# potsawee/tokenize-audio

Hardware: AMD Instinct MI355X
Metric: audio-sec encoded/sec (Mimi 8-codebook, 24 kHz) (higher is better)
Workload: dtype f16x3 (fp32-emulating: 2 fp16 planes per operand, 3 products, fp32 accumulate; RVQ distances fp32); 1 GPU; LibriTTS-R-style batch encode (configs[1]): batch=32 x 10 s @ 24 kHz resident in HBM, K=8 codebooks, 1 encode per step per GPU; global_batch=32, num_quantizers=8, parallelism=utterance round-robin x1 (no collective), gemm_precision=f16x3

## Files before the change

tokenize-audio_amd/csrc/engine.cpp:

```cpp
#include <hip/hip_runtime.h>

#include <algorithm>
#include <cmath>
#include <cstdarg>
#include <cstdio>
#include <cstdlib>
#include <cstring>
#include <fstream>
#include <map>
#include <memory>
#include <mutex>
#include <string>
#include <tuple>
#include <unordered_map>
#include <vector>

#include "../../include/mimi_hip.h"
#include "host_io.h"
#include "kernels.h"

using namespace mimi;

static thread_local std::string g_last_error;

// ... 242 lines not shown
        int ws_gen = 0, rope_gen = 0;
        hipGraph_t g = nullptr;
        hipGraphExec_t x = nullptr;
        uint64_t used = 0;
        unsigned* chain_flag = nullptr;
        size_t chain_clear = 0;
    };
    static constexpr int kMaxGraphs = 8;
    struct Lane {
        void* ws = nullptr;
        size_t ws_bytes = 0;
        int ws_gen = 0;
        hipEvent_t ws_free = nullptr;
        unsigned* amax_dev = nullptr;
        unsigned* amax_red = nullptr;
        void** io_dev = nullptr;
        std::vector<Graph> graphs;
        std::map<std::tuple<int, int64_t, int>, int> graph_seen;
        hipStream_t stream = nullptr;
        hipEvent_t in_ready = nullptr;
        int tickets = 0;
        int64_t encodes = 0;
        bool excl = false;
    };
    static constexpr int kLanes = 2;
    Lane lanes[kLanes];
    Lane* ln = &lanes[0];
    int lanes_opt = 1;
    bool graphs_enabled = true;
    bool capturing = false;
    size_t cap_chain_clear = 0;
    hipStream_t cap_stream = nullptr;
    int rope_gen = 0;
    uint64_t graph_clock = 0;
    int64_t graph_replays = 0, graph_captures = 0;

    bool taps = false;
    int stage0_fused = 1;
    int ln_fused = 1;
    int rvq_form = 0;
    int ln_rpw = 1;
    int rvq_xcd = 1;
    int rvq_chain = 1;
    bool chain_ok = false;
    unsigned* chain_flag = nullptr;
    int rvq_chain_fault = 0;
    int64_t chain_reruns = 0;
    int qkv_attn = 1;
    int qkv_attn_xcd = 1;
    int attn_band_split = 1;
    int sc1_out = 2;
    int fc1_cg = 1;
    int gemm256 = 3;
    int res1_form = 1;
    int res1_stream = 1;
    struct Tap {
        float* d = nullptr;
        size_t cap = 0;
        int64_t dims[3] = {0, 0, 0};
    };
    std::map<std::string, Tap> tapmap;

    bool decode_enabled = false;
    DevConv dec_first, dec_last;
    std::vector<DevConv> dec_up;
    std::vector<DevConv> dec_res3, dec_res1;
    std::vector<DevXfmr> dxf;
    float* outproj = nullptr;
    float* upsample_w = nullptr;
    void* dws = nullptr;
    size_t dws_bytes = 0;
    unsigned* dec_flag = nullptr;
    unsigned* dec_flag_host = nullptr;
};

static int dev_alloc(mimi_engine* e, void** p, size_t bytes) {
    hipError_t err = hipMalloc(p, bytes);
    if (err != hipSuccess) {
        (void)hipGetLastError();
        return set_err(err == hipErrorOutOfMemory ? MIMI_ERR_OUT_OF_MEMORY : MIMI_ERR_HIP, "hipMalloc(%zu): %s",
                       bytes, hipGetErrorString(err));
    }
    e->allocations.push_back(*p);
    return MIMI_OK;
}

static int upload(mimi_engine* e, float** dst, const std::vector<float>& host) {
    int rc = dev_alloc(e, reinterpret_cast<void**>(dst), host.size() * sizeof(float));
    if (rc) return rc;
    HIP_TRY(hipMemcpy(*dst, host.data(), host.size() * sizeof(float), hipMemcpyHostToDevice));
    return MIMI_OK;
}

static uint16_t f2bf_rne(float f) {
    uint32_t u;
    std::memcpy(&u, &f, 4);
    u += 0x7FFF + ((u >> 16) & 1);
    return (uint16_t)(u >> 16);
}
static float bf2f(uint16_t h) {
    const uint32_t u = (uint32_t)h << 16;
    float f;
    std::memcpy(&f, &u, 4);
    return f;
}

// ... 1002 lines not shown
                ra.hamax = ha.amax;
            }
            if (si == 1 && h16) {
                const Act xa = new_act("s1.x"), ha = new_act("s1.h");
                ra.wh16 = e->res1_h16;
                ra.xscale = xa.scale;
                ra.hscale = ha.scale;
                ra.unscale1 = 1.0f / (xa.scale * e->res1_wsc[0]);
                ra.unscale2 = 1.0f / (ha.scale * e->res1_wsc[1]);
                ra.xamax = xa.amax;
                ra.hamax = ha.amax;
                ra.form = e->res1_form;
            }
            if (rg && !(h16 && (si == 0 || si == 1))) return set_err(MIMI_ERR_UNSUPPORTED, "ragged: fp16 blocks only");
            const double H = C / c.compress;
            const double BT = rows_of(si, (double)B * T);
            const double fl = 2.0 * BT * (3.0 * C * H + H * C) + (si == 0 ? 2.0 * BT * C * c.kernel_size : 0.0);
            const DevConv& dc0 = e->down[0];
            bool t1_ceil = p.T[1] == (T + 3) / 4;
            if (rg)
                for (int b = 0; b < B; ++b) t1_ceil = t1_ceil && rg->plan[b].T[1] == (rg->plan[b].T[0] + 3) / 4;
            if (si == 0 && h16 && e->stage0_fused && C == 64 && dc0.cin == 64 && dc0.cout == 128 &&
                dc0.k == 8 && dc0.stride == 4 && dc0.wh && dc0.b && t1_ceil) {
                ra.wdown = dc0.wh;
                ra.bdown = dc0.b;
                ra.unscale_d = 1.0f / (yact.scale * dc0.wscale);
                ra.xout = w.x;
                ra.T1 = p.T[1];
                ra.yp = e->taps ? w.y : nullptr;
                LAUNCH_TRY(launch_stage0_fused(ra, s, &kname), "stage 0 + down conv 0");
                const double BT1 = rows_of(1, (double)B * p.T[1]);
                const double fld = 2.0 * BT1 * 128.0 * 512.0;
                const double by = BT * 4 + BT1 * 128 * 4 + (3.0 * C * H + H * C) * 4 + 128.0 * 512 * 4;
                rec.mark("res_down_s0", fl + fld, by, kname);
                if ((rc = save_tap_planes(e, "res0_elu", w.y, ns, B, T, C, s, yact.scale))) return rc;
                if ((rc = save_tap_planes(e, "down0", w.x, 0, B, p.T[1], 2 * C, s, 0.0f))) return rc;
                C *= 2;
                continue;
            }
            LAUNCH_TRY(launch_resblock(C, ra, s, &kname), "resblock");
            snprintf(nm, sizeof nm, "res_s%d", si);
            const double by = BT * 4 * (si == 0 ? 1 + C : 2 * C) + (3.0 * C * H + H * C) * 4;
            rec.mark(nm, fl, by, kname);
        } else {
            const int Hh = C / c.compress;
            GemmArgs a3 = conv_args(e->res3[si], nullptr, T, nullptr, T, B);
            planes_in(a3, w.xe, (long long)B * T * C);
            use_h(a3, e->res3[si].wh, e->res3[si].wscale, xeact);
            a3.Cp = w.h;
            a3.c_pstride = (long long)B * T * Hh;
            if (rg) a3.a_rows = a3.m_rows = dT[si];
            hact = new_act(nmf("h%d", si));
            out_act(a3, hact);
            LAUNCH_TRY(launch_gemm(ROLE_RES3P, a3, s, &kname, prec), "res3");
            snprintf(nm, sizeof nm, "res3_s%d", si);
            rec.mark(nm, gemm_flops(a3) * rows_of(si, (double)B * T) / ((double)B * T), gemm_bytes(a3, false), kname);
            GemmArgs a1 = conv_args(e->res1[si], nullptr, T, nullptr, T, B);
            planes_in(a1, w.h, (long long)B * T * Hh);
            use_h(a1, e->res1[si].wh, e->res1[si].wscale, hact);
            a1.R = w.x;
            a1.Cp = w.y;
            a1.c_pstride = (long long)B * T * C;
            if (rg) a1.a_rows = a1.m_rows = dT[si];
            yact = new_act(nmf("y%d", si));
            out_act(a1, yact);
            if (h16 && e->res1_stream && res1_stream_ok(a1) && (e->res1_stream == 2 || a1.K == 128))
                LAUNCH_TRY(launch_res1_stream(a1, s, &kname), "res1 stream");
            else
                LAUNCH_TRY(launch_gemm(ROLE_RES1P, a1, s, &kname, prec), "res1");
            snprintf(nm, sizeof nm, "res1_s%d", si);
            rec.mark(nm, gemm_flops(a1) * rows_of(si, (double)B * T) / ((double)B * T), gemm_bytes(a1, true), kname);
        }
        snprintf(nm, sizeof nm, "res%d_elu", si);
        if ((rc = save_tap_planes(e, nm, w.y, ns, B, T, C, s, yact.scale))) return rc;
        const bool last = si == c.num_ratios - 1;
        const bool next_unf = ns && !last && si + 1 >= mimi_engine::kUnfuseFrom;
        GemmArgs ad = conv_args(e->down[si], w.y, T, w.x, p.T[si + 1], B);
        int role = last ? ROLE_DOWN_ELU : ROLE_DOWN;
        if (ns) {
            planes_in(ad, w.y, (long long)B * T * C);
            use_h(ad, e->down[si].wh, e->down[si].wscale, yact);
            if (last) {
                ad.Cp = w.x;
                ad.c_pstride = (long long)B * p.T[si + 1] * 2 * C;
                ad.C = nullptr;
                xact = new_act("x_last");
                out_act(ad, xact);
            } else if (next_unf) {
                ad.Cp = w.xe;
                ad.c_pstride = (long long)B * p.T[si + 1] * 2 * C;
                role = ROLE_DOWN_XE;
                xeact = new_act(nmf("xe%d", si + 1));
                out_act(ad, xeact);
            }
        }
        if (rg) {
            ad.a_rows = dT[si];
            ad.m_rows = dT[si + 1];
        }
        LAUNCH_TRY(launch_gemm(role, ad, s, &kname, prec, rg ? 0 : e->gemm256), "down");
        snprintf(nm, sizeof nm, "down_s%d", si);
        rec.mark(nm, gemm_flops(ad) * rows_of(si + 1, (double)B * p.T[si + 1]) / ((double)B * p.T[si + 1]),
                 gemm_bytes(ad, false), kname);
        snprintf(nm, sizeof nm, last ? "down%d_elu" : "down%d", si);
        if ((rc = save_tap_planes(e, nm, w.x, last ? ns : 0, B, p.T[si + 1], 2 * C, s, last ? xact.scale : 0.0f)))
            return rc;
        C *= 2;
    }
    const int64_t T = p.frames25;
    const int Hd = c.hidden_size;
    GemmArgs af = conv_args(e->final_conv, w.x, p.T[c.num_ratios], w.t0, T, B);
    if (ns) planes_in(af, w.x, (long long)B * p.T[c.num_ratios] * C);
    use_h(af, e->final_conv.wh, e->final_conv.wscale, xact);
    if (rg) {
        af.a_rows = dT[c.num_ratios];
        af.m_rows = dT25;
        af.c_boff = dToff;
    }
    LAUNCH_TRY(launch_gemm(ROLE_FINAL, af, s, &kname, prec), "final");
    const double rT25 = rows_of(5, (double)B * p.frames25) / ((double)B * p.frames25);
    rec.mark("final", gemm_flops(af) * rT25, gemm_bytes(af, false), kname);
    const int64_t rows = rg ? rg->R : (int64_t)B * T;
    const int64_t tapB = rg ? 1 : B, tapT = rg ? rg->R : T;
    if ((rc = save_tap(e, "encoder", w.t0, tapB, tapT, Hd, s))) return rc;
    const int H = c.num_attention_heads, Dh = c.head_dim;
    const bool ds_planes = h16 && e->ds_fix && e->inproj_h && c.downsample_kernel == 4 && c.downsample_stride == 2;
    Act dsin, dsouta;
    double att_flops = 0;
    auto att_fl = [&](int64_t Tn) {
        double f = 0;
        for (int64_t i = 0; i < Tn; ++i) f += 4.0 * Dh * std::min<int64_t>(i + 1, c.sliding_window);
        return f * H;
    };
    if (rg) {
        for (const auto& pb : rg->plan) att_flops += att_fl(pb.frames25);
    } else {
        att_flops = att_fl(T) * B;
    }
    for (int l = 0; l < c.num_hidden_layers; ++l) {
        const DevXfmr& x = e->xf[l];
        const long long nact = rows * Hd;
        Act t1a = new_act(nmf("xf%d.ln1", l));
        if (ln_check_free(t1a, x.ln1_bound)) t1a.amax = nullptr;
        auto ln_into = [&](GemmArgs& g, int role, const float* lw, const float* lb, const Act& act) {
            if (!h16 || e->ln_fused < (role == ROLE_QKV ? 2 : 1) || !gemm_ln_prologue_ok(role, g, prec, rg ? 0 : e->gemm256)) return false;
            if (role == ROLE_QKV) g.ln_tile = e->ln_fused - 2;
            g.ln_x = w.t0;
            g.ln_g = lw;
            g.ln_b = lb;
            g.ln_eps = c.norm_eps;
            g.ln_scale = act.scale;
            g.ln_amax = act.amax;
            return true;
// ... 1394 lines not shown
    delete e;
}

extern "C" int mimi_set_precision(mimi_engine* e, int32_t mode) {
    if (!e) return set_err(MIMI_ERR_INVALID_ARGUMENT, "null engine");
    if (mode < MIMI_PRECISION_F32 || mode > MIMI_PRECISION_F16X3)
        return set_err(MIMI_ERR_INVALID_ARGUMENT, "precision mode %d", mode);
    std::lock_guard<std::mutex> lk(e->mu);
    if (e->precision != mode) {
        HIP_TRY(hipSetDevice(e->device));
        drain_lanes(e);
    }
    e->precision = mode;
    return MIMI_OK;
}

extern "C" int mimi_set_graphs(mimi_engine* e, int32_t enable) {
    if (!e) return set_err(MIMI_ERR_INVALID_ARGUMENT, "null engine");
    std::lock_guard<std::mutex> lk(e->mu);
    HIP_TRY(hipSetDevice(e->device));
    e->graphs_enabled = enable != 0;
    if (!enable) drop_graphs(e, true);
    return MIMI_OK;
}

extern "C" int64_t mimi_graph_replays(const mimi_engine* e) { return e ? e->graph_replays : -1; }

extern "C" int64_t mimi_graph_captures(const mimi_engine* e) { return e ? e->graph_captures : -1; }

extern "C" int64_t mimi_lane_encodes(const mimi_engine* e, int32_t lane) {
    return e && lane >= 0 && lane < mimi_engine::kLanes ? e->lanes[lane].encodes : -1;
}

struct EngineOption {
    const char* key;
    int mimi_engine::*field;
    unsigned allowed;
    const char* values;
};
static const EngineOption kEngineOptions[] = {
    {"stage0_fused", &mimi_engine::stage0_fused, 0x3u, "0 or 1"},
    {"rvq_form", &mimi_engine::rvq_form, 0x7fu, "0..6"},
    {"ln_rpw", &mimi_engine::ln_rpw, 0x117u, "0, 1, 2, 4 or 8"},
    {"rvq_xcd", &mimi_engine::rvq_xcd, 0x3u, "0 or 1"},
    {"rvq_chain", &mimi_engine::rvq_chain, 0x3u, "0 or 1"},
    {"rvq_chain_fault", &mimi_engine::rvq_chain_fault, 0x7u, "0, 1 or 2"},
    {"sc1_out", &mimi_engine::sc1_out, 0xffu, "0..7"},
    {"ln_fused", &mimi_engine::ln_fused, 0x1fu, "0 .. 4"},
    {"qkv_attn", &mimi_engine::qkv_attn, 0x7u, "0, 1 or 2"},
    {"qkv_attn_xcd", &mimi_engine::qkv_attn_xcd, 0x3u, "0 or 1"},
    {"attn_band_split", &mimi_engine::attn_band_split, 0x7u, "0, 1 or 2"},
    {"fc1_cg", &mimi_engine::fc1_cg, 0x17u, "0, 1, 2 or 4"},
    {"gemm256", &mimi_engine::gemm256, 0xffu, "0..7"},
    {"res1_form", &mimi_engine::res1_form, 0x3u, "0 or 1"},
    {"res1_stream", &mimi_engine::res1_stream, 0x7u, "0, 1 or 2"},
    {"lanes", &mimi_engine::lanes_opt, 0x7u, "0, 1 or 2"},
};

extern "C" int mimi_set_option(mimi_engine* e, const char* key, int64_t value) {
    if (!e || !key) return set_err(MIMI_ERR_INVALID_ARGUMENT, "null engine or key");
    std::lock_guard<std::mutex> lk(e->mu);
    for (const EngineOption& o : kEngineOptions) {
        if (strcmp(key, o.key)) continue;
        if (value < 0 || value > 31 || !((o.allowed >> value) & 1u))
            return set_err(MIMI_ERR_INVALID_ARGUMENT, "%s %lld (%s)", key, (long long)value, o.values);
        HIP_TRY(hipSetDevice(e->device));
        drain_lanes(e);
        if (e->*o.field != (int)value) drop_graphs(e, true);
        e->*o.field = (int)value;
        return MIMI_OK;
    }
    return set_err(MIMI_ERR_INVALID_ARGUMENT, "unknown option '%s'", key);
}

extern "C" int mimi_act_scales(mimi_engine* e, int32_t max_n, char* names, float* scales, float* last_max,
                               int32_t* n) {
    if (!e) return set_err(MIMI_ERR_INVALID_ARGUMENT, "null engine");
    std::lock_guard<std::mutex> lk(e->mu);
    int i = 0;
    for (const auto& kv : e->slot_of) {
        const int slot = kv.second;
        if (i >= max_n) break;
        if (names) {
            std::strncpy(names + 64 * i, kv.first.c_str(), 63);
            names[64 * i + 63] = 0;
        }
        if (scales) scales[i] = slot < (int)e->act_scale.size() ? e->act_scale[slot] : 0.0f;
        if (last_max) last_max[i] = slot < (int)e->last_amax.size() ? e->last_amax[slot] : -1.0f;
        ++i;
    }
    if (n) *n = i;
    return MIMI_OK;
}

extern "C" int mimi_get_precision(const mimi_engine* e) { return e ? e->precision : -1; }

extern "C" int mimi_calibrate(mimi_engine* e) {
    if (!e) return set_err(MIMI_ERR_INVALID_ARGUMENT, "null engine");
    if (!e->finalized) return set_err(MIMI_ERR_STATE, "mimi_finalize has not been called");
    std::lock_guard<std::mutex> lk(e->mu);
    if (e->calibrated) return MIMI_OK;
    HIP_TRY(hipSetDevice(e->device));
    (void)hipGetLastError();
    return calibrate_scales(e);
}

// ... 117 lines not shown
```

tokenize-audio_amd/csrc/gemm.hip:

```cpp
#include <algorithm>
#include <cstdio>
#include <cstdlib>


#include "gemm_planes.h"
#include "gemm_planes256.h"

#ifndef MIMI_QKV_V
#define MIMI_QKV_V 1
#endif
#ifndef MIMI_FC1_V
#define MIMI_FC1_V 0
#endif
#ifndef MIMI_SMALL16_32W
#define MIMI_SMALL16_32W 1
#endif
#ifndef MIMI_SMALL16_32
#define MIMI_SMALL16_32 15
#endif


namespace mimi {

template <int BM, int BN, int WM, int WN, int BK, int NBUF, bool NFAST, bool ELU_IN, int PAD, int EPI, int TAG>
// ... 210 lines not shown
            return run_planes<32, 32, 1, 2, 2, MIMI_DOWN_SMALL_ST, EPI, OUTP, TAG, 4, 32, 16, FL_PAIR | FL_KG2, true>(a, s);
        return run_planes<64, 64, 2, 2, 2, 4, EPI, OUTP, TAG, 4, 32, 16, FL_PAIR | FL_KG2, true>(a, s);
    }
    if (pair_ok(a) && tiles(a, 256, 128) < kSmallGrid)
        return run_planes<64, 64, 2, 2, 2, MIMI_DOWN_SMALL2_ST, EPI, OUTP, TAG, 4, 32, 16, FL_PAIR, true>(a, s);
    constexpr int PF = OUTP == 0 ? FL_PF : 0;
    if (pair_ok(a)) return run_planes<256, 128, 4, 2, 2, 2, EPI, OUTP, TAG, 4, 32, 16, FL_PAIR | FL_PERSIST | PF, true>(a, s);
    return run_planes<256, 128, 4, 2, 2, 3, EPI, OUTP, TAG, 0, 32, 16, 0, true>(a, s);
}

#ifndef MIMI_SMALL_ST
#define MIMI_SMALL_ST 4
#endif
#ifndef MIMI_LNA_ST
#define MIMI_LNA_ST 4
#endif
template <int EPI, int OUTP, int TAG, int BN0, int BM1, int BN1, int WM1, int WN1, int BN2, int WN2, int ST = MIMI_SMALL_ST,
          int FL = 0, int BM0 = 64, int WN0 = 2>
static hipError_t run_small_h16(const GemmArgs& a, hipStream_t s) {
    if (tiles(a, BM0, BN0) >= 256) return run_planes<BM0, BN0, 2, WN0, 2, ST, EPI, OUTP, TAG, 4, 32, 16, FL, true>(a, s);
    if (tiles(a, BM1, BN1) >= 256) return run_planes<BM1, BN1, WM1, WN1, 2, ST, EPI, OUTP, TAG, 4, 32, 16, FL, true>(a, s);
    return run_planes<16, BN2, 1, WN2, 2, ST, EPI, OUTP, TAG, 4, 32, 16, FL, true>(a, s);
}

bool gemm_ln_prologue_ok(int role, const GemmArgs& a, int precision, int g256) {
    if (role == ROLE_FC1 && (g256 & 4)) return false;
    return precision == PREC_F16X3 && (role == ROLE_QKV || role == ROLE_FC1) && a.K == 512 && a.a_rs == 512 &&
           a.a_off == 0 && !a.a_rows && !a.m_rows && !a.a_boff && tiles(a, 128, 128) < kSmallGrid;
}

static hipError_t dispatch_planes(int role, const GemmArgs& a, hipStream_t s) {
    const int prec = g_prec;
    if (prec != PREC_BF16X6 && prec != PREC_BF16X3 && prec != PREC_F16X3) return hipErrorInvalidValue;
    if (a.ln_x) {
        if (!gemm_ln_prologue_ok(role, a, prec) || !a.ln_g || !a.ln_b || !(a.ln_scale > 0.0f)) return hipErrorInvalidValue;
        if (role == ROLE_QKV) {
            if (tiles(a, 32, 128) >= 256) return run_planes<32, 128, 2, 2, 2, MIMI_LNA_ST, EPI_ROPE, 0, 5, 4, 32, 16, FL_LNA, true>(a, s);
            if (a.ln_tile == 1) return run_planes<32, 64, 2, 1, 2, MIMI_LNA_ST, EPI_ROPE, 0, 5, 4, 32, 16, FL_LNA, true>(a, s);
            if (a.ln_tile == 2) return run_planes<16, 128, 1, 2, 2, MIMI_LNA_ST, EPI_ROPE, 0, 5, 4, 32, 16, FL_LNA, true>(a, s);
            return run_planes<16, 64, 1, 1, 2, MIMI_LNA_ST, EPI_ROPE, 0, 5, 4, 32, 16, FL_LNA, true>(a, s);
        }
        if (tiles(a, 64, 64) >= 256) return run_planes<64, 64, 2, 2, 2, MIMI_LNA_ST, EPI_GELU, 2, 7, 4, 32, 16, FL_LNA, true>(a, s);
        if (tiles(a, 32, 64) >= 256) return run_planes<32, 64, 2, 2, 2, MIMI_LNA_ST, EPI_GELU, 2, 7, 4, 32, 16, FL_LNA, true>(a, s);
        return run_planes<16, 64, 1, 2, 2, MIMI_LNA_ST, EPI_GELU, 2, 7, 4, 32, 16, FL_LNA, true>(a, s);
    }
    if (prec == PREC_F16X3 && g_g256 && planes256_ok(a)) {
        const bool force = (g_g256 & 4) != 0;
        const bool grid_ok = force || (tiles(a, 256, 256) >= kGrid256 && a.N >= 256);
        if (role == ROLE_FC1 && (force || (g_g256 & 1)) && grid_ok && a.Cp) {
            if (a.sc1) return run_planes256<EPI_GELU, 2, 7, FL_SC1OUT>(a, s);
            return run_planes256<EPI_GELU, 2, 7, 0>(a, s);
        }
        if ((role == ROLE_DOWN || role == ROLE_DOWN_XE) && (force || (g_g256 & 2)) && grid_ok && pair_ok(a)) {
            if (role == ROLE_DOWN) return run_planes256<EPI_BIAS, 0, 2, FL_PAIR | FL_PERSIST>(a, s);
            return run_planes256<EPI_BIAS, 2 | 8, 11, FL_PAIR | FL_PERSIST>(a, s);
        }
    }
#ifndef MIMI_SMALL_ROLES
#define MIMI_SMALL_ROLES 1
#endif
    const bool qsmall = tiles(a, 128, 128) < 256 &&
                        (((MIMI_SMALL_ROLES & 1) && (role == ROLE_DOWNSAMPLE || role == ROLE_INPROJ)) ||
                         ((MIMI_SMALL_ROLES & 2) && role == ROLE_OPROJ) || ((MIMI_SMALL_ROLES & 4) && role == ROLE_FC2) ||
                         ((MIMI_SMALL_ROLES & 8) && role == ROLE_FINAL));
    if (prec == PREC_F16X3 && (tiles(a, 128, 128) < kSmallGrid || qsmall)) {
        switch (role) {
            case ROLE_FINAL:
                if (MIMI_SMALL16_32 & 2) return run_small_h16<EPI_BIAS_OUT, 0, 4, 64, 32, 64, 2, 2, 32, MIMI_SMALL16_32W>(a, s);
                return run_small_h16<EPI_BIAS_OUT, 0, 4, 64, 32, 64, 2, 2, 64, 2>(a, s);
            case ROLE_QKV: return run_small_h16<EPI_ROPE, 0, 5, 128, 32, 128, 2, 2, 64, 1>(a, s);
            case ROLE_OPROJ:
                if (MIMI_SMALL16_32 & 1) return run_small_h16<EPI_SCALE_RES, 0, 6, 64, 32, 64, 2, 2, 32, MIMI_SMALL16_32W>(a, s);
                return run_small_h16<EPI_SCALE_RES, 0, 6, 64, 32, 64, 2, 2, 64, 2>(a, s);
            case ROLE_FC1: return run_small_h16<EPI_GELU, 2, 7, 64, 32, 64, 2, 2, 64, 2>(a, s);
            case ROLE_FC2:
                if (a.Cp)
                    return run_small_h16<EPI_SCALE_RES, 2, 8, 32, 32, 32, 1, 2, 32, MIMI_SMALL16_32W, 6, FL_KG2>(a, s);
                return run_small_h16<EPI_SCALE_RES, 0, 8, 32, 32, 32, 1, 2, 32, MIMI_SMALL16_32W, 6, FL_KG2>(a, s);
            case ROLE_DOWNSAMPLE:
                if (MIMI_SMALL16_32 & 4) return run_small_h16<EPI_NONE, 2, 9, 64, 32, 64, 2, 2, 32, MIMI_SMALL16_32W>(a, s);
                return run_small_h16<EPI_NONE, 2, 9, 64, 32, 64, 2, 2, 64, 2>(a, s);
            case ROLE_INPROJ:
                if (MIMI_SMALL16_32 & 8) return run_small_h16<EPI_NONE, 0, 10, 64, 32, 64, 2, 2, 32, MIMI_SMALL16_32W>(a, s);
                return run_small_h16<EPI_NONE, 0, 10, 64, 32, 64, 2, 2, 64, 2>(a, s);
            case ROLE_RES3P: return run_small_h16<EPI_BIAS_ELU, 2, 12, 64, 32, 64, 2, 2, 64, 2, 3>(a, s);
            default: break;
        }
    }
    if (prec == PREC_F16X3) {
        switch (role) {
            case ROLE_FC2:
                if (a.Cp) return run_planes<128, 128, 4, 2, 2, 3, EPI_SCALE_RES, 2, 8, 4, 32, 16, 0, true>(a, s);
                break;
            case ROLE_DOWNSAMPLE: return run_planes<128, 128, 4, 2, 2, 2, EPI_NONE, 2, 9, 0, 32, 16, 0, true>(a, s);
            case ROLE_INPROJ: return run_planes<128, 128, 4, 2, 2, 2, EPI_NONE, 0, 10, 0, 32, 16, 0, true>(a, s);
            default: break;
        }
        switch (role) {
            case ROLE_DOWN: return run_planes_down_h16<EPI_BIAS, 0, 2>(a, s);
            case ROLE_DOWN_ELU: return run_planes_down_h16<EPI_BIAS_ELU, 2, 3>(a, s);
            case ROLE_DOWN_XE: return run_planes_down_h16<EPI_BIAS, 2 | 8, 11>(a, s);
            default: break;
        }
    }
    switch (role) {
        case ROLE_DOWN: return run_planes_big<EPI_BIAS, 0, 0, 2>(a, s, prec);
        case ROLE_DOWN_ELU: return run_planes_big_ld<EPI_BIAS_ELU, 3, 2, 3>(a, s, prec);
        case ROLE_FINAL: return run_planes_small_ld<EPI_BIAS_OUT, 4>(a, s, prec);
        case ROLE_QKV:
// ... 70 lines not shown
```

tokenize-audio_amd/csrc/gemm_planes.h:

```cpp
#pragma once
#include <type_traits>

#include "gemm_kernel.h"

namespace mimi {

#if defined(__HIP_DEVICE_COMPILE__)
__device__ __forceinline__ __amdgpu_buffer_rsrc_t make_rsrc(const void* base, long long bytes) {
    const long long lim = bytes < 0x7fffffffLL ? bytes : 0x7fffffffLL;
    return __builtin_amdgcn_make_buffer_rsrc(const_cast<void*>(base), (short)0, (int)lim, 0x00020000);
}
#endif

template <int PM, int L>
__device__ __forceinline__ void wait_stages(int later) {
    if constexpr (L == 0) {
        asm volatile("s_waitcnt vmcnt(0)" ::: "memory");
    } else {
        if (later >= L)
            asm volatile("s_waitcnt vmcnt(%0)" ::"n"(L * PM) : "memory");
        else
            wait_stages<PM, L - 1>(later);
    }
}

__device__ __forceinline__ int xcd_remap(int bid, int nwg) {
    const int xcd = bid & 7, q = nwg >> 3, r = nwg & 7;
    return (xcd < r ? xcd * (q + 1) : r * (q + 1) + (xcd - r) * q) + (bid >> 3);
}

template <int BK, int MF>
__device__ __forceinline__ int chunk_swz(int row) {
    if (BK == 16) return (row >> 3) & 1;
    if (MF == 16) return ((row >> 3) & 1) * 3;
    return (row >> 2) & 3;
}


enum : int { FL_PRIO = 2, FL_PAIR = 4, FL_PERSIST = 8, FL_KG2 = 16, FL_KG4 = 32, FL_PF = 256, FL_RAGGED = 512,
             FL_LNA = 2048, FL_SC1OUT = 4096 };
enum : int { FL_DIAG_NODMA = 64, FL_DIAG_NOMMA = 128 };
enum : int { FL_DIAG_ILV = 1024 };

template <int BM, int BN, int WM, int WN, int NS, int STAGES, int EPI, int OUTP, int TAG, int LW = 0, int BK = 32,
          int MF = 32, int FL = 0, bool F16 = false>
__global__ __launch_bounds__((WM * WN + LW) * 64) void gemm_planes_kernel(GemmArgs p) {
#if defined(__HIP_DEVICE_COMPILE__)
    constexpr int NW = WM * WN;
    constexpr int NLD = LW > 0 ? LW : NW;
    constexpr int CPR = BK / 8;
    constexpr int RPP = 64 / CPR;
    constexpr int TM = BM / WM / MF;
    constexpr int TN = BN / WN / MF;
    constexpr int KSUB = MF == 32 ? BK / 16 : BK / 32;
    constexpr bool PAIR = (FL & FL_PAIR) != 0;
    constexpr int KG = (FL & FL_KG4) ? 4 : (FL & FL_KG2) ? 2 : 1;
    constexpr int XR = PAIR ? RPP : 0;
    constexpr int NB = PAIR ? 2 : 1;
    constexpr int AR = BM + XR;
    constexpr int APL = AR * BK, BPL = BN * BK;
    constexpr bool LNA = (FL & FL_LNA) != 0;
    constexpr int BOFF = LNA ? 0 : NS * APL;
    constexpr int STG = BOFF + NS * NB * BPL;
    constexpr int TPA = LNA ? 0 : NS * AR / RPP, TP = TPA + NS * NB * BN / RPP;
    constexpr int PMAX = (TP + NLD - 1) / NLD;
    constexpr int PMIN = TP / NLD;
    static_assert(BK == 32 || (BK == 16 && MF == 32), "BK");
    static_assert(MF == 32 || MF == 16, "MFMA shape");
    static_assert(TM >= 1 && TN >= 1 && KSUB >= 1, "tile");
    static_assert(NS * BM % RPP == 0 && NS * BN % RPP == 0, "whole pieces");
    static_assert(STAGES >= 2 * KG && STAGES <= 16, "stages");
    static_assert(PMAX * (STAGES - 2 * KG) <= 63, "vmcnt range");
    static_assert(EPI != EPI_ROPE || (MF == 32 ? TN % 2 == 0 : TN % 4 == 0), "rope pairs (d, d+32) in one lane");
    static_assert(!F16 || NS == 2, "fp16 planes: 2 planes, 3 products");
    static_assert(!LNA || (F16 && !PAIR && !(FL & (FL_PERSIST | FL_RAGGED | FL_DIAG_ILV))), "LayerNorm prologue");
    constexpr int LNK = 512;
    constexpr int LNE = LNA ? LNK / BK * NS * APL : 0;
    constexpr int ONS = OUTP & 7;
    typedef typename std::conditional<MF == 32, f32x16, f32x4>::type accT;
    constexpr int NACC = MF == 32 ? 16 : 4;

    constexpr int CW = TN * MF, RW = TM * MF;
    constexpr int PFS0 = (STAGES - KG) * STG;
    constexpr bool PFIT1 = PFS0 * 2 + NW * RW * (CW + 4) * 4 <= 160 * 1024;
    constexpr bool PFIT2 = TN % 2 == 0 && PFS0 * 2 + NW * RW * (CW / 2 + 4) * 4 <= 160 * 1024;
    constexpr bool PFIT4 = TN % 4 == 0 && PFS0 * 2 + NW * RW * (CW / 4 + 4) * 4 <= 160 * 1024;
    constexpr bool PF = (FL & FL_PF) && (FL & FL_PERSIST) && LW > 0 && (PFIT1 || PFIT2 || PFIT4);
    constexpr int PFS = PF ? PFS0 : 0;
    constexpr int JH = PF ? (PFIT1 ? 1 : PFIT2 ? 2 : 4) : (NW * RW * (CW + 4) * 4 <= 160 * 1024 ? 1 : 2);
    constexpr int TNC = TN / JH, CWC = TNC * MF, LDE = CWC + 4;
    static_assert(TNC * JH == TN, "epilogue passes");
    constexpr int LDS_EL = STAGES * STG > PFS + NW * RW * LDE * 2 ? STAGES * STG : PFS + NW * RW * LDE * 2;
    static_assert((LDS_EL + LNE) * 2 <= 160 * 1024, "LDS");
    __shared__ __attribute__((aligned(16))) __bf16 lds[LDS_EL + LNE];

// ... 409 lines not shown
```

tokenize-audio_amd/csrc/gemm_planes256.h:

```cpp
#pragma once
#include "gemm_planes.h"

namespace mimi {

template <int EPI, int OUTP, int TAG, int FL = 0>
__global__ __launch_bounds__(512) void gemm_planes256_kernel(GemmArgs p) {
#if defined(__HIP_DEVICE_COMPILE__)
    constexpr int BM = 256, BN = 256, BK = 32, MF = 16, NW = 8;
    constexpr int TM = 8, TN = 4;
    constexpr int PL = 128 * BK;
    constexpr int HT = 2 * PL;
    constexpr int RING = 8 * HT;
    constexpr bool PAIR = (FL & FL_PAIR) != 0;
    constexpr int ONS = OUTP & 7;
    constexpr int JH = 2, LDE = TN * MF / JH + 4;
    constexpr int LDS_EL = RING > NW * TM * MF * LDE * 2 ? RING : NW * TM * MF * LDE * 2;
    static_assert(LDS_EL * 2 <= 160 * 1024, "LDS");
    __shared__ __attribute__((aligned(16))) __bf16 lds[LDS_EL];

    const int tid = threadIdx.x;
    const int lane = tid & 63;
    const int wave = __builtin_amdgcn_readfirstlane(tid >> 6);
    const int wm = wave >> 2, wn = wave & 3;
    const bool late = wave >= 4;
    const int M = p.M, N = p.N, K = p.K;
    const int MT = (M + BM - 1) / BM, NTn = (N + BN - 1) / BN;
    const int ntiles = MT * NTn * p.batch;
    const int KT = K / BK;
    const int NH = 4 * KT;
    const int ncg = (p.ncg > 1 && NTn % p.ncg == 0) ? p.ncg : 1;
    float omx = 0.0f;

    const int prow = wave * 16 + (lane >> 2), pch = lane & 3;
    const int csrc = (pch ^ chunk_swz<BK, MF>(prow)) * 8;
    const int a_trow = (prow >> 6) * 128 + (prow & 63);
    const int b_tcol = (prow >> 5) * 64 + (prow & 31);
    const __bf16* __restrict__ Wp = reinterpret_cast<const __bf16*>(p.Wsplit);
    const int w_pl = N * K;

    const int fr = lane & 15, hsel = lane >> 4;
    const int a_frag = (wm * 64 + fr) * BK + ((hsel ^ chunk_swz<BK, MF>(fr)) * 8);
    const int b_frag = (wn * 32 + fr) * BK + ((hsel ^ chunk_swz<BK, MF>(fr)) * 8);

    for (int tile = blockIdx.x; tile < ntiles; tile += gridDim.x) {
    int b, mt, nt;
    {
        const int logical = xcd_remap(tile, ntiles);
        int rest;
        if (ncg > 1) {
            const int NG = NTn / ncg, per = ntiles / ncg;
            const int cg = logical / per, w = logical - cg * per;
            nt = cg * NG + w % NG;
            rest = w / NG;
        } else {
            nt = logical % NTn;
            rest = logical / NTn;
        }
        mt = __builtin_amdgcn_readfirstlane(rest % MT);
        b = __builtin_amdgcn_readfirstlane(rest / MT);
        nt = __builtin_amdgcn_readfirstlane(nt);
    }
    const int m0 = mt * BM, n0 = nt * BN;
    const __bf16* __restrict__ Abase = reinterpret_cast<const __bf16*>(p.Ap) + (long long)b * p.a_bstride;
    const __amdgpu_buffer_rsrc_t ars0 = make_rsrc(Abase, p.a_len * 2);
    const __amdgpu_buffer_rsrc_t ars1 = make_rsrc(Abase + p.a_pstride, p.a_len * 2);
    int a_src[2], b_src[2];
#pragma unroll
    for (int h = 0; h < 2; ++h) {
        const int m = m0 + a_trow + h * 64;
        a_src[h] = m < M ? (int)((p.a_off + (long long)m * p.a_rs + csrc) * 2) : -16;
        int n = n0 + b_tcol + h * 32;
        n = n < N ? n : N - 1;
        b_src[h] = n * K + csrc;
    }

    KOrderT<BK> ko;
    ko.init(p, PAIR);
    const int ktap = PAIR ? ko.s * ko.cin : 0;
    int kstep = 0;
    auto k_of_issue = [&]() {
        return PAIR ? ko.offset() + (kstep & 1) * ktap : ko.offset();
    };
    auto k_advance = [&]() {
        if (!PAIR || (kstep & 1)) ko.next();
        ++kstep;
    };
    auto issue = [&](int slot, auto rc, int k0) {
        constexpr int r = decltype(rc)::value;
        __bf16* dst = lds + (slot * 4 + r) * HT + wave * 16 * BK;
        if constexpr (r & 1) {
            const int off = a_src[r >> 1] + k0 * 2;
            __builtin_amdgcn_raw_ptr_buffer_load_lds(ars0, (__attribute__((address_space(3))) void*)dst, 16, off, 0, 0, 0);
            __builtin_amdgcn_raw_ptr_buffer_load_lds(ars1, (__attribute__((address_space(3))) void*)(dst + PL), 16, off,
                                                     0, 0, 0);
        } else {
            const __bf16* src = Wp + b_src[r >> 1] + k0;
            __builtin_amdgcn_global_load_lds((const void*)src, (__attribute__((address_space(3))) void*)dst, 16, 0, 0);
            __builtin_amdgcn_global_load_lds((const void*)(src + w_pl), (__attribute__((address_space(3))) void*)(dst + PL),
                                             16, 0, 0);
        }
    };

    f32x4 acc[TM][TN];
#pragma unroll
    for (int i = 0; i < TM; ++i)
#pragma unroll
        for (int j = 0; j < TN; ++j)
#pragma unroll
            for (int r = 0; r < 4; ++r) acc[i][j][r] = 0.0f;

    {
        const int k0 = k_of_issue();
        k_advance();
        issue(0, std::integral_constant<int, 0>(), k0);
        issue(0, std::integral_constant<int, 1>(), k0);
        issue(0, std::integral_constant<int, 2>(), k0);
        issue(0, std::integral_constant<int, 3>(), k0);
    }
    int kiss = k_of_issue();
    k_advance();
    issue(1, std::integral_constant<int, 0>(), kiss);
    issue(1, std::integral_constant<int, 1>(), kiss);
    asm volatile("s_waitcnt vmcnt(8)" ::: "memory");
    __builtin_amdgcn_s_barrier();
    if (late) __builtin_amdgcn_s_barrier();
    asm volatile("" ::: "memory");

    bf16x8 af[2][4], bf[2][2][2];
    auto read_a = [&](const __bf16* ht) {
#pragma unroll
        for (int pl = 0; pl < 2; ++pl)
#pragma unroll
            for (int i = 0; i < 4; ++i) af[pl][i] = *reinterpret_cast<const bf16x8*>(ht + pl * PL + a_frag + i * 16 * BK);
    };
    auto read_b = [&](const __bf16* ht, int sb) {
#pragma unroll
        for (int pl = 0; pl < 2; ++pl)
#pragma unroll
            for (int j = 0; j < 2; ++j) bf[sb][pl][j] = *reinterpret_cast<const bf16x8*>(ht + pl * PL + b_frag + j * 16 * BK);
    };
    auto mma_quad = [&](auto sac, auto sbc) {
        constexpr int sa = decltype(sac)::value, sb = decltype(sbc)::value;
        if (FL & FL_DIAG_NOMMA) return;
#pragma unroll
        for (int i = 0; i < 4; ++i)
#pragma unroll
            for (int j = 0; j < 2; ++j) {
                f32x4& c = acc[sa * 4 + i][sb * 2 + j];
                c = mfma16<true>(af[1][i], bf[sb][0][j], c);
                c = mfma16<true>(af[0][i], bf[sb][1][j], c);
                c = mfma16<true>(af[0][i], bf[sb][0][j], c);
            }
    };
    auto phase_tail = [&](int pphase, int slot_iss, auto rc, auto sac, auto sbc) {
        const int h = pphase + 6;
        if (!(FL & FL_DIAG_NODMA) && h < NH) issue(slot_iss, rc, kiss);
        wait_stages<2, 4>(min(4, max(0, NH - 3 - pphase)));
        __builtin_amdgcn_s_barrier();
        asm volatile("s_waitcnt lgkmcnt(0)" ::: "memory");
        __builtin_amdgcn_sched_barrier(0);
        __builtin_amdgcn_s_setprio(1);
        mma_quad(sac, sbc);
        __builtin_amdgcn_s_setprio(0);
        __builtin_amdgcn_sched_barrier(0);
        __builtin_amdgcn_s_barrier();
        asm volatile("" ::: "memory");
    };
    using I0 = std::integral_constant<int, 0>;
    using I1 = std::integral_constant<int, 1>;
    using I2 = std::integral_constant<int, 2>;
    using I3 = std::integral_constant<int, 3>;

    for (int kt = 0; kt < KT; ++kt) {
        const __bf16* st = lds + (kt & 1) * 4 * HT;
        const int s1 = (kt + 1) & 1, s2 = kt & 1;
        const int p0 = 4 * kt;
        read_b(st + 0 * HT, 0);
        __builtin_amdgcn_sched_barrier(0);
        read_a(st + 1 * HT);
        asm volatile("" ::: "memory");
        phase_tail(p0 + 0, s1, I2(), I0(), I0());
        read_b(st + 2 * HT, 1);
        asm volatile("" ::: "memory");
        phase_tail(p0 + 1, s1, I3(), I0(), I1());
        read_a(st + 3 * HT);
        asm volatile("" ::: "memory");
        if (kt + 2 < KT) {
            kiss = k_of_issue();
            k_advance();
        }
        phase_tail(p0 + 2, s2, I0(), I1(), I1());
        phase_tail(p0 + 3, s2, I1(), I1(), I0());
    }
    if (!late) __builtin_amdgcn_s_barrier();

    __syncthreads();
    {
    constexpr bool F16 = true;
    float* stg = reinterpret_cast<float*>(lds) + wave * (TM * MF * LDE);
    const long long cel = (long long)b * p.c_bstride;
    const int rbase = m0 + wm * TM * MF, cb0 = n0 + wn * TN * MF;
    const int Mb = M;
#include "gemm_planes_epilogue.inc"
    }
    if (FL & FL_PERSIST) {
        asm volatile("s_waitcnt lgkmcnt(0)" ::: "memory");
        __builtin_amdgcn_s_barrier();
    }
    }
    if (ONS) amax_commit(p.out_amax, omx);
#endif
}

}
```

Baseline: 55120 audio-sec/sec.

## Share A tiles across paired conv taps in 256 GEMM via halo rows

Adds a FL_SHARE mode to the 256-tile planes GEMM for the downsample conv pair order. The second tap reuses the first tap's A rows shifted by one, reading from LDS plus a small halo row loaded by one wave, so it no longer issues its own global A load. This needs a reworked vmcnt wait schedule and a new swizzle for A. It is enabled by default for the down GEMMs through g256_share=1. Separately, there is an opt-in (off by default) option to route the res3 GEMM through the 256 kernel.

Result: no change. 55380 audio-sec/sec (median of 6 runs) (+0.5%).

```diff
diff --git a/tokenize-audio_amd/csrc/engine.cpp b/tokenize-audio_amd/csrc/engine.cpp
--- a/tokenize-audio_amd/csrc/engine.cpp
+++ b/tokenize-audio_amd/csrc/engine.cpp
@@ -318,6 +318,8 @@
     int sc1_out = 2;
     int fc1_cg = 1;
     int gemm256 = 3;
+    int g256_res3 = 0;
+    int g256_share = 1;
     int res1_form = 1;
     int res1_stream = 1;
     struct Tap {
@@ -1426,7 +1428,8 @@
             if (rg) a3.a_rows = a3.m_rows = dT[si];
             hact = new_act(nmf("h%d", si));
             out_act(a3, hact);
-            LAUNCH_TRY(launch_gemm(ROLE_RES3P, a3, s, &kname, prec), "res3");
+            const int g3 = rg || !e->gemm256 || !e->g256_res3 ? 0 : e->gemm256 | (e->g256_res3 == 2 ? 16 : 8);
+            LAUNCH_TRY(launch_gemm(ROLE_RES3P, a3, s, &kname, prec, g3), "res3");
             snprintf(nm, sizeof nm, "res3_s%d", si);
             rec.mark(nm, gemm_flops(a3) * rows_of(si, (double)B * T) / ((double)B * T), gemm_bytes(a3, false), kname);
             GemmArgs a1 = conv_args(e->res1[si], nullptr, T, nullptr, T, B);
@@ -1472,7 +1475,7 @@
             ad.a_rows = dT[si];
             ad.m_rows = dT[si + 1];
         }
-        LAUNCH_TRY(launch_gemm(role, ad, s, &kname, prec, rg ? 0 : e->gemm256), "down");
+        LAUNCH_TRY(launch_gemm(role, ad, s, &kname, prec, rg || !e->gemm256 ? 0 : e->gemm256 | (e->g256_share ? 32 : 0)), "down");
         snprintf(nm, sizeof nm, "down_s%d", si);
         rec.mark(nm, gemm_flops(ad) * rows_of(si + 1, (double)B * p.T[si + 1]) / ((double)B * p.T[si + 1]),
                  gemm_bytes(ad, false), kname);
@@ -2973,6 +2976,8 @@
     {"attn_band_split", &mimi_engine::attn_band_split, 0x7u, "0, 1 or 2"},
     {"fc1_cg", &mimi_engine::fc1_cg, 0x17u, "0, 1, 2 or 4"},
     {"gemm256", &mimi_engine::gemm256, 0xffu, "0..7"},
+    {"g256_res3", &mimi_engine::g256_res3, 0x7u, "0, 1 or 2"},
+    {"g256_share", &mimi_engine::g256_share, 0x3u, "0 or 1"},
     {"res1_form", &mimi_engine::res1_form, 0x3u, "0 or 1"},
     {"res1_stream", &mimi_engine::res1_stream, 0x7u, "0, 1 or 2"},
     {"lanes", &mimi_engine::lanes_opt, 0x7u, "0, 1 or 2"},
diff --git a/tokenize-audio_amd/csrc/gemm.hip b/tokenize-audio_amd/csrc/gemm.hip
--- a/tokenize-audio_amd/csrc/gemm.hip
+++ b/tokenize-audio_amd/csrc/gemm.hip
@@ -286,9 +286,16 @@
             return run_planes256<EPI_GELU, 2, 7, 0>(a, s);
         }
         if ((role == ROLE_DOWN || role == ROLE_DOWN_XE) && (force || (g_g256 & 2)) && grid_ok && pair_ok(a)) {
+            if (g_g256 & 32) {
+                if (role == ROLE_DOWN) return run_planes256<EPI_BIAS, 0, 2, FL_PAIR | FL_PERSIST | FL_SHARE>(a, s);
+                return run_planes256<EPI_BIAS, 2 | 8, 11, FL_PAIR | FL_PERSIST | FL_SHARE>(a, s);
+            }
             if (role == ROLE_DOWN) return run_planes256<EPI_BIAS, 0, 2, FL_PAIR | FL_PERSIST>(a, s);
             return run_planes256<EPI_BIAS, 2 | 8, 11, FL_PAIR | FL_PERSIST>(a, s);
         }
+        if (role == ROLE_RES3P && (g_g256 & (8 | 16)) && a.N >= 256 && a.Cp &&
+            ((g_g256 & 16) || tiles(a, 256, 256) >= kGrid256))
+            return run_planes256<EPI_BIAS_ELU, 2, 12, 0>(a, s);
     }
 #ifndef MIMI_SMALL_ROLES
 #define MIMI_SMALL_ROLES 1
diff --git a/tokenize-audio_amd/csrc/gemm_planes.h b/tokenize-audio_amd/csrc/gemm_planes.h
--- a/tokenize-audio_amd/csrc/gemm_planes.h
+++ b/tokenize-audio_amd/csrc/gemm_planes.h
@@ -41,6 +41,8 @@
              FL_LNA = 2048, FL_SC1OUT = 4096 };
 enum : int { FL_DIAG_NODMA = 64, FL_DIAG_NOMMA = 128 };
 enum : int { FL_DIAG_ILV = 1024 };
+enum : int { FL_DIAG_NOSHA = 8192 };
+enum : int { FL_SHARE = 16384 };
 
 template <int BM, int BN, int WM, int WN, int NS, int STAGES, int EPI, int OUTP, int TAG, int LW = 0, int BK = 32,
           int MF = 32, int FL = 0, bool F16 = false>
diff --git a/tokenize-audio_amd/csrc/gemm_planes256.h b/tokenize-audio_amd/csrc/gemm_planes256.h
--- a/tokenize-audio_amd/csrc/gemm_planes256.h
+++ b/tokenize-audio_amd/csrc/gemm_planes256.h
@@ -1,5 +1,6 @@
 #pragma once
 #include "gemm_planes.h"
+#include "ring_wait.h"
 
 namespace mimi {
 
@@ -12,10 +13,14 @@
     constexpr int HT = 2 * PL;
     constexpr int RING = 8 * HT;
     constexpr bool PAIR = (FL & FL_PAIR) != 0;
+    constexpr bool SHARE = (FL & FL_SHARE) != 0;
+    static_assert(!SHARE || (PAIR && !(FL & FL_DIAG_NOSHA)), "FL_SHARE: the pair order only");
     constexpr int ONS = OUTP & 7;
     constexpr int JH = 2, LDE = TN * MF / JH + 4;
     constexpr int LDS_EL = RING > NW * TM * MF * LDE * 2 ? RING : NW * TM * MF * LDE * 2;
     static_assert(LDS_EL * 2 <= 160 * 1024, "LDS");
+    constexpr int HALO = 512;
+    static_assert(!SHARE || (RING + PL + 2 * HALO <= LDS_EL && 2 * HALO <= PL), "halo rows behind the ring");
     __shared__ __attribute__((aligned(16))) __bf16 lds[LDS_EL];
 
     const int tid = threadIdx.x;
@@ -23,6 +28,7 @@
     const int wave = __builtin_amdgcn_readfirstlane(tid >> 6);
     const int wm = wave >> 2, wn = wave & 3;
     const bool late = wave >= 4;
+    const bool halo_wave = wave == 7;
     const int M = p.M, N = p.N, K = p.K;
     const int MT = (M + BM - 1) / BM, NTn = (N + BN - 1) / BN;
     const int ntiles = MT * NTn * p.batch;
@@ -33,14 +39,18 @@
 
     const int prow = wave * 16 + (lane >> 2), pch = lane & 3;
     const int csrc = (pch ^ chunk_swz<BK, MF>(prow)) * 8;
+#define MIMI_A_SWZ(row) (SHARE ? (((row) >> 2) & 1) * 2 : chunk_swz<BK, MF>(row))
+    const int csrc_a = (pch ^ MIMI_A_SWZ(prow)) * 8;
     const int a_trow = (prow >> 6) * 128 + (prow & 63);
     const int b_tcol = (prow >> 5) * 64 + (prow & 31);
     const __bf16* __restrict__ Wp = reinterpret_cast<const __bf16*>(p.Wsplit);
     const int w_pl = N * K;
 
     const int fr = lane & 15, hsel = lane >> 4;
-    const int a_frag = (wm * 64 + fr) * BK + ((hsel ^ chunk_swz<BK, MF>(fr)) * 8);
+    const int a_frag = (wm * 64 + fr) * BK + ((hsel ^ MIMI_A_SWZ(fr)) * 8);
     const int b_frag = (wn * 32 + fr) * BK + ((hsel ^ chunk_swz<BK, MF>(fr)) * 8);
+    const int a_sh = (wm * 64 + fr + 1) * BK + ((hsel ^ MIMI_A_SWZ(fr + 1)) * 8);
+#undef MIMI_A_SWZ
 
     for (int tile = blockIdx.x; tile < ntiles; tile += gridDim.x) {
     int b, mt, nt;
@@ -68,11 +78,14 @@
 #pragma unroll
     for (int h = 0; h < 2; ++h) {
         const int m = m0 + a_trow + h * 64;
-        a_src[h] = m < M ? (int)((p.a_off + (long long)m * p.a_rs + csrc) * 2) : -16;
+        a_src[h] = m < M + (SHARE ? 1 : 0) ? (int)((p.a_off + (long long)m * p.a_rs + csrc_a) * 2) : -16;
         int n = n0 + b_tcol + h * 32;
         n = n < N ? n : N - 1;
         b_src[h] = n * K + csrc;
     }
+
+    int halo_src = (int)0x80000000u;
+    if (SHARE && lane < 4 && m0 + 255 < M) halo_src = (int)((p.a_off + (long long)(m0 + 256) * p.a_rs + lane * 8) * 2);
 
     KOrderT<BK> ko;
     ko.init(p, PAIR);
@@ -81,14 +94,19 @@
     auto k_of_issue = [&]() {
         return PAIR ? ko.offset() + (kstep & 1) * ktap : ko.offset();
     };
+    auto sha_of_issue = [&]() {
+        return PAIR ? (kstep & 1) != 0 : ko.c > 0;
+    };
     auto k_advance = [&]() {
         if (!PAIR || (kstep & 1)) ko.next();
         ++kstep;
     };
+    bool kiss_sha = false;
     auto issue = [&](int slot, auto rc, int k0) {
         constexpr int r = decltype(rc)::value;
         __bf16* dst = lds + (slot * 4 + r) * HT + wave * 16 * BK;
         if constexpr (r & 1) {
+            if ((FL & FL_DIAG_NOSHA) && kiss_sha) return;
             const int off = a_src[r >> 1] + k0 * 2;
             __builtin_amdgcn_raw_ptr_buffer_load_lds(ars0, (__attribute__((address_space(3))) void*)dst, 16, off, 0, 0, 0);
             __builtin_amdgcn_raw_ptr_buffer_load_lds(ars1, (__attribute__((address_space(3))) void*)(dst + PL), 16, off,
@@ -101,6 +119,19 @@
         }
     };
 
+    auto issue_halo = [&](int set, int k0) {
+        __bf16* dst = lds + RING + set * HALO;
+        const int off = halo_src + k0 * 2;
+        __builtin_amdgcn_raw_ptr_buffer_load_lds(ars0, (__attribute__((address_space(3))) void*)dst, 16, off, 0, 0, 0);
+        __builtin_amdgcn_raw_ptr_buffer_load_lds(ars1, (__attribute__((address_space(3))) void*)(dst + PL), 16, off, 0, 0, 0);
+    };
+    auto cnt = [&](int h) {
+        if (h >= NH) return 0;
+        if (!(h & 1)) return 2;
+        if (h & 4) return 0;
+        return (h & 2) && halo_wave ? 4 : 2;
+    };
+
     f32x4 acc[TM][TN];
 #pragma unroll
     for (int i = 0; i < TM; ++i)
@@ -116,12 +147,18 @@
         issue(0, std::integral_constant<int, 1>(), k0);
         issue(0, std::integral_constant<int, 2>(), k0);
         issue(0, std::integral_constant<int, 3>(), k0);
+        if (SHARE && halo_wave) issue_halo(0, k0);
     }
     int kiss = k_of_issue();
+    kiss_sha = sha_of_issue();
     k_advance();
     issue(1, std::integral_constant<int, 0>(), kiss);
-    issue(1, std::integral_constant<int, 1>(), kiss);
-    asm volatile("s_waitcnt vmcnt(8)" ::: "memory");
+    if constexpr (SHARE) {
+        vm_wait(cnt(2) + cnt(3) + cnt(4) + cnt(5));
+    } else {
+        issue(1, std::integral_constant<int, 1>(), kiss);
+        asm volatile("s_waitcnt vmcnt(8)" ::: "memory");
+    }
     __builtin_amdgcn_s_barrier();
     if (late) __builtin_amdgcn_s_barrier();
     asm volatile("" ::: "memory");
@@ -132,6 +169,19 @@
         for (int pl = 0; pl < 2; ++pl)
 #pragma unroll
             for (int i = 0; i < 4; ++i) af[pl][i] = *reinterpret_cast<const bf16x8*>(ht + pl * PL + a_frag + i * 16 * BK);
+    };
+    auto read_a_sh = [&](int set, auto sac) {
+        constexpr int sa = decltype(sac)::value;
+        const int base = (set * 4 + 1 + 2 * sa) * HT;
+        int o3 = sa == 0 ? (set * 4 + 3) * HT + wm * 64 * BK : (wm == 0 ? (set * 4 + 1) * HT + 64 * BK : RING + set * HALO);
+        o3 = fr == 15 ? o3 + hsel * 8 : base + a_sh + 3 * 16 * BK;
+#pragma unroll
+        for (int pl = 0; pl < 2; ++pl) {
+#pragma unroll
+            for (int i = 0; i < 3; ++i)
+                af[pl][i] = *reinterpret_cast<const bf16x8*>(lds + base + pl * PL + a_sh + i * 16 * BK);
+            af[pl][3] = *reinterpret_cast<const bf16x8*>(lds + pl * PL + o3);
+        }
     };
     auto read_b = [&](const __bf16* ht, int sb) {
 #pragma unroll
@@ -152,10 +202,33 @@
                 c = mfma16<true>(af[0][i], bf[sb][0][j], c);
             }
     };
-    auto phase_tail = [&](int pphase, int slot_iss, auto rc, auto sac, auto sbc) {
+    auto phase_tail = [&](int pphase, int slot_iss, auto rc, auto sac, auto sbc, auto parc) {
         const int h = pphase + 6;
-        if (!(FL & FL_DIAG_NODMA) && h < NH) issue(slot_iss, rc, kiss);
-        wait_stages<2, 4>(min(4, max(0, NH - 3 - pphase)));
+        if constexpr (SHARE) {
+            constexpr int r = decltype(rc)::value, par = decltype(parc)::value;
+            constexpr int q = (r + 2) & 3;
+            constexpr bool a_iss = (r & 1) && (q == 1 ? par == 1 : par == 0);
+            const int aset = (h >> 3) & 1;
+            if constexpr (!(r & 1) || a_iss) {
+                if (!(FL & FL_DIAG_NODMA) && h < NH) {
+                    issue((r & 1) ? aset : slot_iss, rc, kiss);
+                    if (r == 3 && halo_wave) issue_halo(aset, kiss);
+                }
+            }
+            constexpr int n0 = par == 0 ? (q == 0 || q == 3 ? 6 : 4) : (q == 0 || q == 3 ? 6 : 8);
+            constexpr bool nx = par == 0 ? q == 0 : q != 0;
+            if (h < NH) {
+                if (nx && halo_wave)
+                    asm volatile("s_waitcnt vmcnt(%0)" ::"n"(n0 + 2) : "memory");
+                else
+                    asm volatile("s_waitcnt vmcnt(%0)" ::"n"(n0) : "memory");
+            } else {
+                vm_wait(cnt(pphase + 3) + cnt(pphase + 4) + cnt(pphase + 5) + cnt(pphase + 6));
+            }
+        } else {
+            if (!(FL & FL_DIAG_NODMA) && h < NH) issue(slot_iss, rc, kiss);
+            wait_stages<2, 4>(min(4, max(0, NH - 3 - pphase)));
+        }
         __builtin_amdgcn_s_barrier();
         asm volatile("s_waitcnt lgkmcnt(0)" ::: "memory");
         __builtin_amdgcn_sched_barrier(0);
@@ -171,26 +244,44 @@
     using I2 = std::integral_constant<int, 2>;
     using I3 = std::integral_constant<int, 3>;
 
-    for (int kt = 0; kt < KT; ++kt) {
+    auto k_step = [&](int kt, auto parc) {
+        constexpr bool tap2 = decltype(parc)::value == 1;
         const __bf16* st = lds + (kt & 1) * 4 * HT;
         const int s1 = (kt + 1) & 1, s2 = kt & 1;
         const int p0 = 4 * kt;
+        const int aset = (kt >> 1) & 1;
+        const __bf16* sta = SHARE ? lds + aset * 4 * HT : st;
         read_b(st + 0 * HT, 0);
         __builtin_amdgcn_sched_barrier(0);
-        read_a(st + 1 * HT);
+        if constexpr (tap2)
+            read_a_sh(aset, I0());
+        else
+            read_a(sta + 1 * HT);
         asm volatile("" ::: "memory");
-        phase_tail(p0 + 0, s1, I2(), I0(), I0());
+        phase_tail(p0 + 0, s1, I2(), I0(), I0(), parc);
         read_b(st + 2 * HT, 1);
         asm volatile("" ::: "memory");
-        phase_tail(p0 + 1, s1, I3(), I0(), I1());
-        read_a(st + 3 * HT);
+        phase_tail(p0 + 1, s1, I3(), I0(), I1(), parc);
+        if constexpr (tap2)
+            read_a_sh(aset, I1());
+        else
+            read_a(sta + 3 * HT);
         asm volatile("" ::: "memory");
         if (kt + 2 < KT) {
             kiss = k_of_issue();
+            kiss_sha = sha_of_issue();
             k_advance();
         }
-        phase_tail(p0 + 2, s2, I0(), I1(), I1());
-        phase_tail(p0 + 3, s2, I1(), I1(), I0());
+        phase_tail(p0 + 2, s2, I0(), I1(), I1(), parc);
+        phase_tail(p0 + 3, s2, I1(), I1(), I0(), parc);
+    };
+    if constexpr (SHARE) {
+        for (int kt = 0; kt < KT; kt += 2) {
+            k_step(kt, I0());
+            k_step(kt + 1, I1());
+        }
+    } else {
+        for (int kt = 0; kt < KT; ++kt) k_step(kt, std::integral_constant<int, -1>());
     }
     if (!late) __builtin_amdgcn_s_barrier();
 
```
